# kan-bayashi/espnet

Measured on AMD Instinct MI355X. Metric: frames/sec, 12L Conformer hybrid CTC/attention training step (B=32 T=1000 d=256 per GPU), higher is better.
Workload: dtype f32; 1 GPU; BASELINE configs[1]: 12L Conformer enc d=256 h=4 ff=2048 k=31 macaron+cnn rel_pos, 6L Transformer dec, V=5000, fbank B=32 T=1000 L=100, mtlalpha 0.3, lsm 0.1; global_batch=32, frames=1000, parallelism=dp1, optimizer=adam+noam, clip 5.0, launch=hipGraph, wgrad_side_stream=False, optimizer_steps_done=113

## Files before the change

### espnet_amd/csrc/convmod.hip

```cpp
#include <stdlib.h>
#include "common.h"
#include "../../include/espnet_amd.h"

namespace {

constexpr int KMAX = 32;

__device__ __forceinline__ void chan_merge(float& n, float& mean, float& m2, float nb, float mb, float m2b);

template <int NWV, int MODE>
__global__ __launch_bounds__(NWV * 64) void dwconv_lds_kernel(const float* __restrict__ x, const float* __restrict__ w,
                                                              const float* __restrict__ bias, float* __restrict__ y,
                                                              int B, int T, int C, int K, int pad, int flip,
                                                              const float* __restrict__ aglu, int y_bf16,
                                                              float* __restrict__ bn_part) {
  constexpr int TB = NWV * 8;
  constexpr int NR = (TB + KMAX - 1 + NWV - 1) / NWV;
  constexpr int NWL = (64 * KMAX + NWV * 64 - 1) / (NWV * 64);
  __shared__ float xs[(TB + KMAX - 1) * 64];
  __shared__ float wl[64 * KMAX];
  const int lane = threadIdx.x & 63, wave = threadIdx.x >> 6;
  const int c0 = blockIdx.x * 64;
  const int c = min(c0 + lane, C - 1);
  const int nblk = (T + TB - 1) / TB;
// ... 169 lines not shown
  __syncthreads();
  float* slot = smem + wave * 64 * (KMAX + 1);
#pragma unroll
  for (int k = 0; k < KMAX; ++k)
    if (k < K) slot[lane * (KMAX + 1) + k] = live ? acc[k] : 0.f;
  redb[wave * 64 + lane] = live ? accb : 0.f;
  __syncthreads();
  const int nch = min(64, C - c0);
  for (int i = threadIdx.x; i < nch * K; i += blockDim.x) {
    const int cc = i / K, k = i % K;
    float t = 0.f;
#pragma unroll
    for (int wv = 0; wv < NWV; ++wv) t += smem[wv * 64 * (KMAX + 1) + cc * (KMAX + 1) + k];
    atomicAdd(&dw[(long)c0 * K + i], t);
  }
  if (db && threadIdx.x < nch) {
    float t = 0.f;
#pragma unroll
    for (int wv = 0; wv < NWV; ++wv) t += redb[wv * 64 + threadIdx.x];
    atomicAdd(&db[c0 + threadIdx.x], t);
  }
}

constexpr int BN_R = 4;
struct BnGeom { int cq, rs, slab_rows; };
__host__ __device__ inline BnGeom bn_geom(int C) {
  BnGeom g;
  g.cq = C / 4;
  g.rs = 256 / g.cq;
  g.slab_rows = BN_R * g.rs;
  return g;
}
__device__ __forceinline__ void chan_merge(float& n, float& mean, float& m2, float nb, float mb, float m2b) {
  const float nt = n + nb;
  if (nt > 0.f) {
    const float d = mb - mean;
    const float f = nb / nt;
    mean += d * f;
    m2 += m2b + d * d * n * f;
  }
  n = nt;
}

__global__ __launch_bounds__(256) void bn_partial_kernel(const float* __restrict__ x, float* __restrict__ part,
                                                         long M, int C, int T, const int* __restrict__ bound) {
  __shared__ float4 sh_mean[256], sh_m2[256];
// ... 82 lines not shown
      chan_merge(n, mean, m2, sh[0][o], sh[1][o], sh[2][o]);
    }
    const float var = m2 / n;
    mean_out[c] = mean;
    rstd_out[c] = rsqrtf(var + eps);
    if (running_mean) {
      running_mean[c] = (1.f - momentum) * running_mean[c] + momentum * mean;
      running_var[c] = (1.f - momentum) * running_var[c] + momentum * (n > 1.f ? m2 / (n - 1.f) : var);
    }
  }
}
__global__ void bn_apply_kernel(const float* __restrict__ x, const float* __restrict__ mean,
                                const float* __restrict__ rstd, const float* __restrict__ gamma,
                                const float* __restrict__ beta, float* __restrict__ y, long M, int C, int act,
                                int bf16) {
  const long n = M * C;
  const long stride = (long)gridDim.x * blockDim.x;
  unsigned short* y16 = reinterpret_cast<unsigned short*>(y);
  for (long i = (long)blockIdx.x * blockDim.x + threadIdx.x; i < n; i += stride) {
    int c = i % C;
    float z = (x[i] - mean[c]) * rstd[c] * gamma[c] + beta[c];
    z = eamd_act(z, act);
    if (bf16) y16[i] = eamd_f2bf(z); else y[i] = z;
  }
}
__global__ __launch_bounds__(256) void bn_bwd_partial_kernel(const float* __restrict__ dy, const float* __restrict__ x,
                                                             const float* __restrict__ mean,
                                                             const float* __restrict__ rstd,
                                                             const float* __restrict__ gamma,
                                                             const float* __restrict__ beta, float* __restrict__ part,
                                                             long M, int C, int act, int T,
                                                             const int* __restrict__ bound) {
  __shared__ float4 sh1[256], sh2[256];
  const int tb = bound ? bound[0] : T;
  const BnGeom g = bn_geom(C);
  const int t = threadIdx.x;
  const int q = t % g.cq, sub = t / g.cq;
  const bool live = sub < g.rs;
  const long r0 = (long)blockIdx.x * g.slab_rows + sub;
  float4 mu = make_float4(0.f, 0.f, 0.f, 0.f), rs = mu, gm = mu, be = mu;
  if (live) {
    mu = reinterpret_cast<const float4*>(mean)[q]; rs = reinterpret_cast<const float4*>(rstd)[q];
    gm = reinterpret_cast<const float4*>(gamma)[q]; be = reinterpret_cast<const float4*>(beta)[q];
  }
  float4 xv[BN_R], dv[BN_R];
#pragma unroll
// ... 261 lines not shown
  }
  red[sub][lane] = (s0 + s1) + (s2 + s3);
  __syncthreads();
  if (sub == 0 && col < 10 * C) {
    const float v = (red[0][lane] + red[1][lane]) + (red[2][lane] + red[3][lane]);
    const int k = col / C, c = col % C;
    if (k < 9) atomicAdd(&dw[(long)c * 9 + k], v); else atomicAdd(&db[c], v);
  }
}

inline int grid_for(long n) {
  long b = (n + 255) / 256;
  if (b < 1) b = 1;
  if (b > 4096) b = 4096;
  return (int)b;
}

inline void dwconv_launch(const float* x, const float* w, const float* bias, float* y, int B, int T, int C, int K,
                          int flip, hipStream_t s) {
  hipLaunchKernelGGL((dwconv_lds_kernel<8, 0>), dim3((C + 63) / 64, B * ((T + 63) / 64)), dim3(512), 0, s, x, w, bias, y, B, T, C,
                     K, (K - 1) / 2, flip, (const float*)nullptr, 0, (float*)nullptr);
}

}

extern "C" {

int eamd_dwconv_fwd(const float* x, const float* w, const float* bias, float* y, int B, int T, int C, int K,
                    void* stream) {
  if (!x || !w || !y || B <= 0 || T <= 0 || C <= 0 || K <= 0 || (K & 1) == 0) return EAMD_EINVAL;
  if (K > KMAX) return EAMD_EUNSUPPORTED;
  dwconv_launch(x, w, bias, y, B, T, C, K, 0, (hipStream_t)stream);
  EAMD_LAUNCH_CHECK();
  return EAMD_OK;
}

int eamd_dwconv_bwd_x(const float* dy, const float* w, float* dx, int B, int T, int C, int K, void* stream) {
  if (!dy || !w || !dx || B <= 0 || T <= 0 || C <= 0 || K <= 0 || (K & 1) == 0) return EAMD_EINVAL;
  if (K > KMAX) return EAMD_EUNSUPPORTED;
  dwconv_launch(dy, w, (const float*)nullptr, dx, B, T, C, K, 1, (hipStream_t)stream);
  EAMD_LAUNCH_CHECK();
  return EAMD_OK;
}

int eamd_dwconv_bwd_w(const float* dy, const float* x, float* dw, float* db, int B, int T, int C, int K,
                      void* stream) {
  if (!dy || !x || !dw || B <= 0 || T <= 0 || C <= 0 || K <= 0 || (K & 1) == 0) return EAMD_EINVAL;
  if (K > KMAX) return EAMD_EUNSUPPORTED;
  const long total = (long)B * ((T + WNWV * 8 - 1) / (WNWV * 8));
  const int gx = (C + 63) / 64;
  long gy = (512 + gx - 1) / gx;
  if (gy > total) gy = total;
  if (gy < 1) gy = 1;
  const long tpb = (total + gy - 1) / gy;
  gy = (total + tpb - 1) / tpb;
  hipLaunchKernelGGL(dwconv_bwd_w_kernel, dim3(gx, (unsigned)gy), dim3(WNWV * 64), 0, (hipStream_t)stream, dy, x, dw, db, B,
                     T, C, K, (K - 1) / 2, (int)tpb, 0);
  EAMD_LAUNCH_CHECK();
  return EAMD_OK;
}

int eamd_dwconv_glu_fwd(const float* a, const float* w, const float* bias, float* y, float* bn_part, int B, int T, int C, int K,
                        void* stream) {
  if (!a || !w || !y || B <= 0 || T <= 0 || C <= 0 || K <= 0 || (K & 1) == 0) return EAMD_EINVAL;
  if (K > KMAX) return EAMD_EUNSUPPORTED;
  hipLaunchKernelGGL((dwconv_lds_kernel<8, 1>), dim3((C + 63) / 64, B * ((T + 63) / 64)), dim3(512), 0, (hipStream_t)stream, a, w,
                     bias, y, B, T, C, K, (K - 1) / 2, 0, (const float*)nullptr, 0, bn_part);
  EAMD_LAUNCH_CHECK();
  return EAMD_OK;
}

int eamd_dwconv_glu_bwd_x(const float* dy, const float* w, const float* a, void* da, int da_bf16, int B, int T, int C, int K,
                          void* stream) {
  if (!dy || !w || !a || !da || B <= 0 || T <= 0 || C <= 0 || K <= 0 || (K & 1) == 0) return EAMD_EINVAL;
  if (K > KMAX) return EAMD_EUNSUPPORTED;
  hipLaunchKernelGGL((dwconv_lds_kernel<8, 2>), dim3((C + 63) / 64, B * ((T + 63) / 64)), dim3(512), 0, (hipStream_t)stream, dy, w,
                     (const float*)nullptr, (float*)da, B, T, C, K, (K - 1) / 2, 1, a, da_bf16, (float*)nullptr);
  EAMD_LAUNCH_CHECK();
  return EAMD_OK;
}

int eamd_dwconv_glu_bwd_w(const float* dy, const float* a, float* dw, float* db, int B, int T, int C, int K, void* stream) {
  if (!dy || !a || !dw || B <= 0 || T <= 0 || C <= 0 || K <= 0 || (K & 1) == 0) return EAMD_EINVAL;
  if (K > KMAX) return EAMD_EUNSUPPORTED;
  const long total = (long)B * ((T + WNWV * 8 - 1) / (WNWV * 8));
  const int gx = (C + 63) / 64;
  long gy = (512 + gx - 1) / gx;
  if (gy > total) gy = total;
  if (gy < 1) gy = 1;
  const long tpb = (total + gy - 1) / gy;
  gy = (total + tpb - 1) / tpb;
  hipLaunchKernelGGL(dwconv_bwd_w_kernel, dim3(gx, (unsigned)gy), dim3(WNWV * 64), 0, (hipStream_t)stream, dy, a, dw, db, B,
                     T, C, K, (K - 1) / 2, (int)tpb, 1);
  EAMD_LAUNCH_CHECK();
  return EAMD_OK;
}

static bool bn_shape_ok(int C) { return C >= 4 && C <= 1024 && C % 4 == 0; }
int eamd_bn_nslab(int64_t M, int C) {
  if (!bn_shape_ok(C) || M <= 0) return 0;
  const BnGeom g = bn_geom(C);
  return (int)((M + g.slab_rows - 1) / g.slab_rows);
}

static int bn_stats_impl(const float* x, float* workspace, float* mean, float* rstd, float* running_mean,
                         float* running_var, int64_t* num_batches_tracked, int64_t M, int C, float eps, float momentum, int T,
                         const int32_t* bound, void* stream) {
  if (!x || !workspace || !mean || !rstd || M <= 0 || C <= 0) return EAMD_EINVAL;
  if (bound && (T <= 0 || M % T != 0)) return EAMD_EINVAL;
  if (!bn_shape_ok(C)) return EAMD_EUNSUPPORTED;
  if ((uintptr_t)x & 15) return EAMD_EINVAL;
  hipStream_t s = (hipStream_t)stream;
  const int nslab = eamd_bn_nslab(M, C);
  hipLaunchKernelGGL(bn_partial_kernel, dim3(nslab), dim3(256), 0, s, x, workspace, (long)M, C, T, (const int*)bound);
  EAMD_LAUNCH_CHECK();
  hipLaunchKernelGGL(bn_finalize_kernel, dim3((C + BN_CPB - 1) / BN_CPB), dim3(1024), 0, s, workspace, nslab, C, eps, momentum, mean, rstd,
                     running_mean, running_var, (long long*)num_batches_tracked);
  EAMD_LAUNCH_CHECK();
// ... 2 lines not shown
int eamd_bn_stats(const float* x, float* workspace, float* mean, float* rstd, float* running_mean,
                  float* running_var, int64_t* num_batches_tracked, int64_t M, int C, float eps, float momentum, void* stream) {
  return bn_stats_impl(x, workspace, mean, rstd, running_mean, running_var, num_batches_tracked, M, C, eps, momentum, 1, nullptr, stream);
}
int eamd_bn_stats_bounded(const float* x, float* workspace, float* mean, float* rstd, float* running_mean,
                          float* running_var, int64_t* num_batches_tracked, int64_t M, int C, float eps, float momentum, int T,
                          const int32_t* bound, void* stream) {
  if (!bound) return EAMD_EINVAL;
  return bn_stats_impl(x, workspace, mean, rstd, running_mean, running_var, num_batches_tracked, M, C, eps, momentum, T, bound, stream);
}

int eamd_bn_finalize(const float* part, int nslab, float* mean, float* rstd, float* running_mean, float* running_var,
                     int64_t* num_batches_tracked, int C, float eps, float momentum, void* stream) {
  if (!part || !mean || !rstd || nslab <= 0 || C <= 0) return EAMD_EINVAL;
  hipLaunchKernelGGL(bn_finalize_kernel, dim3((C + BN_CPB - 1) / BN_CPB), dim3(1024), 0, (hipStream_t)stream, part, nslab, C, eps,
                     momentum, mean, rstd, running_mean, running_var, (long long*)num_batches_tracked);
  EAMD_LAUNCH_CHECK();
  return EAMD_OK;
}

int eamd_bn_apply(const float* x, const float* mean, const float* rstd, const float* gamma, const float* beta,
                  void* y, int64_t M, int C, int act, int y_bf16, void* stream) {
  if (!x || !mean || !rstd || !gamma || !beta || !y || M <= 0 || C <= 0) return EAMD_EINVAL;
  hipLaunchKernelGGL(bn_apply_kernel, dim3(grid_for(M * C)), dim3(256), 0, (hipStream_t)stream, x, mean, rstd, gamma,
                     beta, (float*)y, (long)M, C, act, y_bf16);
  EAMD_LAUNCH_CHECK();
  return EAMD_OK;
}

static int bn_bwd_impl(const float* dy, const float* x, const float* mean, const float* rstd, const float* gamma,
                       const float* beta, float* workspace, float* dx, float* dgamma, float* dbeta, int64_t M, int C,
                       int act, int training, int T, const int32_t* bound, void* stream) {
  if (!dy || !x || !mean || !rstd || !gamma || !beta || !workspace || !dx || !dgamma || !dbeta || M <= 0 || C <= 0)
    return EAMD_EINVAL;
  if (bound && (T <= 0 || M % T != 0)) return EAMD_EINVAL;
  if (!bn_shape_ok(C)) return EAMD_EUNSUPPORTED;
  if (((uintptr_t)x | (uintptr_t)dy | (uintptr_t)mean | (uintptr_t)rstd | (uintptr_t)gamma | (uintptr_t)beta) & 15)
    return EAMD_EINVAL;
  hipStream_t s = (hipStream_t)stream;
  const int nslab = eamd_bn_nslab(M, C);
  float* sums = workspace + (long)nslab * 2 * C;
  hipLaunchKernelGGL(bn_bwd_partial_kernel, dim3(nslab), dim3(256), 0, s, dy, x, mean, rstd, gamma, beta,
                     workspace, (long)M, C, act, T, (const int*)bound);
  EAMD_LAUNCH_CHECK();
  hipLaunchKernelGGL(bn_bwd_finalize_kernel, dim3((C + BN_CPB - 1) / BN_CPB), dim3(1024), 0, s, workspace, nslab, C, sums, dgamma, dbeta);
  EAMD_LAUNCH_CHECK();
  hipLaunchKernelGGL(bn_bwd_apply_kernel, dim3(grid_for(M * C)), dim3(256), 0, s, dy, x, mean, rstd, gamma, beta,
                     sums, dx, (long)M, C, act, training, T, (const int*)bound);
  EAMD_LAUNCH_CHECK();
  return EAMD_OK;
}
int eamd_bn_bwd(const float* dy, const float* x, const float* mean, const float* rstd, const float* gamma,
                const float* beta, float* workspace, float* dx, float* dgamma, float* dbeta, int64_t M, int C,
                int act, int training, void* stream) {
  return bn_bwd_impl(dy, x, mean, rstd, gamma, beta, workspace, dx, dgamma, dbeta, M, C, act, training, 1, nullptr, stream);
}
int eamd_bn_bwd_bounded(const float* dy, const float* x, const float* mean, const float* rstd, const float* gamma,
                        const float* beta, float* workspace, float* dx, float* dgamma, float* dbeta, int64_t M, int C,
                        int act, int training, int T, const int32_t* bound, void* stream) {
  if (!bound) return EAMD_EINVAL;
  return bn_bwd_impl(dy, x, mean, rstd, gamma, beta, workspace, dx, dgamma, dbeta, M, C, act, training, T, bound, stream);
}

static int conv_c1_fwd(const float* x, const float* w, const float* bias, void* y, int B, int T, int F, int C,
                       int y_bf16, int st, int pad, void* stream) {
  if (!x || !w || !bias || !y || B <= 0 || T + 2 * pad < 3 || F + 2 * pad < 3 || C <= 0) return EAMD_EINVAL;
  if (F + 2 * pad > C1_MAXF) return EAMD_EUNSUPPORTED;
  int H = (T + 2 * pad - 3) / st + 1, W = (F + 2 * pad - 3) / st + 1;
  hipStream_t s = (hipStream_t)stream;
  const bool pair = y_bf16 && (C % 2 == 0) && (((uintptr_t)y & 3) == 0);
  const int nthr = pair ? ((C / 2 + 63) / 64) * 64 : 256;
#define EAMD_C1F(ST_, NC_) hipLaunchKernelGGL((conv1_fwd_kernel<ST_, NC_>), dim3(B * H), dim3(min(nthr, 256)), 0, s, x, w, \
                                              bias, (float*)y, B, T, F, H, W, C, y_bf16, pad)
  if (st == 2) { if (pair) EAMD_C1F(2, 2); else EAMD_C1F(2, 1); }
  else         { if (pair) EAMD_C1F(1, 2); else EAMD_C1F(1, 1); }
#undef EAMD_C1F
  EAMD_LAUNCH_CHECK();
  return EAMD_OK;
}
int eamd_conv1_fwd(const float* x, const float* w, const float* bias, void* y, int B, int T, int F, int C,
                   int y_bf16, void* stream) {
  return conv_c1_fwd(x, w, bias, y, B, T, F, C, y_bf16, 2, 0, stream);
}
int eamd_conv3x3_c1_fwd(const float* x, const float* w, const float* bias, void* y, int B, int T, int F, int C,
// ... 64 lines not shown
```

### espnet_amd/functional.py

```python
import math

import torch

from . import ops
from .ops import (ACT_NONE, ACT_RELU, ACT_SWISH, EPI_DACT_FACTOR, EPI_MUL_AUX, EPI_MUL_DSWISH, EPI_MUL_RELU_MASK, EPI_NONE,
                  EPI_RELU)


class GradSink:

    on_done = None
    on_use = None

    @staticmethod
    def use(params):
        if GradSink.on_use is not None and torch.is_grad_enabled():
            GradSink.on_use(params)
        return params

    def __init__(self, params):
        self.params = list(params)
        self.ret = [None] * len(self.params)

    def buf(self, i):
# ... 812 lines not shown
        else:
            dq = ops.to_act(dqu)
        kv_in = mem2 if cross else xn
        ops.linear_bwd_w(dq, xn, sink.buf(2), db=sink.buf(3))
        dxn = ops.linear_bwd_x(dq, ops.wshadow(wq))
        dmem = None
        if pre_kv is not None:
            dx = _ln_bwd_out(dxn, x2, ln_w, mean, rstd, do, sink.buf(0), sink.buf(1), ctx.prev, (B, T1, D))
            return (dx, None, None, None, None, None, None, None, None, None) + sink.results()
        ops.linear_bwd_w(dkk, kv_in, sink.buf(4), db=sink.buf(5))
        ops.linear_bwd_w(dv, kv_in, sink.buf(6), db=sink.buf(7))
        if cross:
            dmem = ops.linear_bwd_x(dkk, ops.wshadow(wk))
            ops.linear_bwd_x(dv, ops.wshadow(wv), out=dmem, beta=1.0)
            dmem = dmem.view(B, T2, D)
        else:
            ops.linear_bwd_x(dkk, ops.wshadow(wk), out=dxn, beta=1.0)
            ops.linear_bwd_x(dv, ops.wshadow(wv), out=dxn, beta=1.0)
        dx = _ln_bwd_out(dxn, x2, ln_w, mean, rstd, do, sink.buf(0), sink.buf(1), ctx.prev, (B, T1, D))
        return (dx, dmem, None, None, None, None, None, None, None, None) + sink.results()


FUSE_GLU_DWCONV = True


class ConvModuleBlockFn(torch.autograd.Function):
    @staticmethod
    def forward(ctx, x, running_mean, running_var, training, act, eps, bn_eps, bn_momentum, drop, *params):
        p_out, s_out = drop
        ln_w, ln_b, w1, b1, wd, bd_, g, be, w2, b2 = params
        B, T, D = x.shape
        Cc = w2.shape[0]
        K = wd.shape[-1]
        M = B * T
        adt = ops.act_dtype()
        x2 = x.reshape(M, D).contiguous()
        rp = None
        if eps is not None and D == 256 and Cc == 256 and x2.dtype == torch.float32 and adt == torch.float32 \
                and ops.rowproj_ok(M, D, 2 * Cc) and (p_out <= 0.0 or ops.f32_epilogue_drop()):
            w1v, w2v = w1.detach().view(2 * Cc, D), w2.detach().view(Cc, Cc)
            rp = ops.rowproj_images(w1, [(w1v, False), (w1v, True), (w2v, False), (w2v, True)])
        if rp is not None:
            xn = torch.empty_like(x2)
            mean = torch.empty(M, device=x2.device, dtype=torch.float32)
            rstd = torch.empty_like(mean)
            a = ops.rowproj(xn, rp[0], 2 * Cc, bias=b1, ln=(x2, ln_w, ln_b, eps, mean, rstd))
# ... 36 lines not shown
        ctx.save_for_backward(x2, mean, rstd, xn, a, gl, d, bmean, brstd, e)
        ctx.pr = GradSink.use(params)
        ctx.cfg = (B, T, D, Cc, K, act, training, drop)
        ctx.bound = bound
        ctx.prev = _prev_drop(x)
        return _tag_out(out.view(B, T, D), p_out, s_out)

    @staticmethod
    def backward(ctx, dout):
        x2, mean, rstd, xn, a, gl, d, bmean, brstd, e = ctx.saved_tensors
        ln_w, ln_b, w1, b1, wd, bd_, g, be, w2, b2 = ctx.pr
        B, T, D, Cc, K, act, training, (p_out, s_out) = ctx.cfg
        M = B * T
        adt = ops.act_dtype()
        sink = GradSink(ctx.pr)
        do = dout.reshape(M, D).contiguous()
        dob = _grad_in(dout, do, p_out, s_out)
        rp = ctx.rp
        ops.linear_bwd_w(dob, e, sink.buf(8).view(Cc, Cc), db=sink.buf(9))
        if rp is not None:
            de = ops.rowproj(dob, rp[3], Cc)
        else:
            de = ops.linear_bwd_x(dob, ops.wshadow(w2).view(Cc, Cc))
        dd = ops.bn_bwd(de, d, bmean, brstd, g, be, sink.buf(6), sink.buf(7), M, Cc, act, training, bound=ctx.bound)
        if gl is None:
            da = ops.dwconv_glu_bwd_x(dd, wd.view(Cc, K), a, B, T, Cc, K, adt)
            if ctx.bound is not None:
                ops.mask_time(da, T, ctx.bound[1])
            ops.dwconv_glu_bwd_w(dd, a, sink.buf(4).view(Cc, K), sink.buf(5), B, T, Cc, K)
        else:
            dgl = ops.dwconv_bwd_x(dd, wd.view(Cc, K), B, T, Cc, K)
            ops.dwconv_bwd_w(dd, gl, sink.buf(4).view(Cc, K), sink.buf(5), B, T, Cc, K)
            da = ops.glu_bwd(dgl, a, Cc, adt)
            if ctx.bound is not None:
                ops.mask_time(da, T, ctx.bound[1])
        ops.linear_bwd_w(da, xn, sink.buf(2).view(2 * Cc, D), db=sink.buf(3))
        if rp is not None and da.dtype == torch.float32:
            dx = _rp_ln_bwd(da, rp[1], x2, ln_w, mean, rstd, do, sink.buf(0), sink.buf(1), ctx.prev, (B, T, D))
        else:
            dxn = ops.linear_bwd_x(da, ops.wshadow(w1).view(2 * Cc, D))
            dx = _ln_bwd_out(dxn, x2, ln_w, mean, rstd, do, sink.buf(0), sink.buf(1), ctx.prev, (B, T, D))
        return (dx, None, None, None, None, None, None, None, None) + sink.results()


_TAPS_FWD = [(kh, kw) for kh in range(3) for kw in range(3)]
_CLASSES = [((0, 0), [(0, 0), (0, 2), (2, 0), (2, 2)]), ((0, 1), [(0, 1), (2, 1)]),
            ((1, 0), [(1, 0), (1, 2)]), ((1, 1), [(1, 1)])]


def _conv3s2_fwd(y_in, w, b, B, Hi, Wi, Cc, adt):
    Ho, Wo = (Hi - 3) // 2 + 1, (Wi - 3) // 2 + 1
    wf, wd = ops.conv2_weight_prep(w, adt)
    g = ops.make_gather(Cc, _TAPS_FWD, Ho, Wo, Hi, Wi, 2, 2)
    M = B * Ho * Wo
    y = torch.empty(M, Cc, device=y_in.device, dtype=adt)
    ops.gemm(y_in, wf, y, M, Cc, 9 * Cc, 9 * Cc, Cc, Cc, transB=1, bias=b, epilogue=EPI_RELU, gather=g)
    return y, wd, Ho, Wo

# ... 337 lines not shown
```

### espnet_amd/ops.py

```python
import ctypes as C
import os
import math

import torch

from . import _lib
from ._lib import GatherT, GemmT, RowMapT, check, ptr, stream_ptr

ACT_NONE, ACT_RELU, ACT_SWISH = 0, 1, 2
EPI_NONE, EPI_RELU, EPI_SWISH, EPI_MUL_RELU_MASK, EPI_MUL_DSWISH, EPI_MUL_AUX, EPI_DACT_FACTOR, EPI_ROW_STATS, EPI_ROW_GRAD = 0, 1, 2, 3, 4, 5, 6, 7, 8

_PRECISIONS = {"fp32": 0, "bf16": 1}
_state = {"precision": 0}


def set_precision(name):
    if name not in _PRECISIONS:
        raise ValueError(f"precision must be one of {list(_PRECISIONS)}")
    _state["precision"] = _PRECISIONS[name]


def get_precision():
    return [k for k, v in _PRECISIONS.items() if v == _state["precision"]][0]

# ... 1690 lines not shown
    if bn is None:
        return y
    eps, momentum, running_mean, running_var, nbt = bn
    mean = torch.empty(Cc, device=a.device, dtype=torch.float32)
    rstd = torch.empty(Cc, device=a.device, dtype=torch.float32)
    check(_lib.lib().eamd_bn_finalize(ptr(part), nslab, ptr(mean), ptr(rstd), ptr(running_mean), ptr(running_var), ptr(nbt), Cc,
                                      eps, momentum, stream_ptr()), "eamd_bn_finalize")
    return y, mean, rstd


def dwconv_glu_bwd_x(dy, w, a, B, T, Cc, K, out_dtype=torch.float32):
    da = torch.empty(a.shape, device=a.device, dtype=out_dtype)
    check(_lib.lib().eamd_dwconv_glu_bwd_x(ptr(dy), ptr(w), ptr(a), ptr(da), int(out_dtype == torch.bfloat16), B, T, Cc, K,
                                           stream_ptr()), "eamd_dwconv_glu_bwd_x")
    return da


def dwconv_glu_bwd_w(dy, a, dw, db, B, T, Cc, K):
    assert dw.numel() == Cc * K and (db is None or db.numel() == Cc)
    check(_lib.lib().eamd_dwconv_glu_bwd_w(ptr(dy), ptr(a), ptr(dw), ptr(db), B, T, Cc, K, stream_ptr()),
          "eamd_dwconv_glu_bwd_w")


def bn_stats(x, M, Cc, eps, momentum, running_mean, running_var, num_batches_tracked=None, bound=None):
    nslab = _lib.lib().eamd_bn_nslab(M, Cc)
    ws = torch.empty(3 * Cc * nslab, device=x.device, dtype=torch.float32)
    mean = torch.empty(Cc, device=x.device, dtype=torch.float32)
    rstd = torch.empty(Cc, device=x.device, dtype=torch.float32)
    assert num_batches_tracked is None or (num_batches_tracked.dtype == torch.int64 and num_batches_tracked.is_cuda)
    if bound is not None:
        check(_lib.lib().eamd_bn_stats_bounded(ptr(x), ptr(ws), ptr(mean), ptr(rstd), ptr(running_mean), ptr(running_var),
                                               ptr(num_batches_tracked), M, Cc, eps, momentum,
                                               int(bound[0]), ptr(bound[1]), stream_ptr()), "eamd_bn_stats_bounded")
        return mean, rstd
    check(_lib.lib().eamd_bn_stats(ptr(x), ptr(ws), ptr(mean), ptr(rstd), ptr(running_mean), ptr(running_var),
                                   ptr(num_batches_tracked), M, Cc, eps, momentum, stream_ptr()),
          "eamd_bn_stats")
    return mean, rstd


def bn_apply(x, mean, rstd, gamma, beta, M, Cc, act, out_dtype=torch.float32):
    y = torch.empty(x.shape, device=x.device, dtype=out_dtype)
    check(_lib.lib().eamd_bn_apply(ptr(x), ptr(mean), ptr(rstd), ptr(gamma), ptr(beta), ptr(y), M, Cc,
                                   act, 1 if out_dtype == torch.bfloat16 else 0, stream_ptr()), "eamd_bn_apply")
    return y

# ... 1285 lines not shown
```

### include/espnet_amd.h

```cpp
#ifndef ESPNET_AMD_H_
#define ESPNET_AMD_H_
#include <stdint.h>
#ifdef __cplusplus
extern "C" {
#endif

int eamd_abi_version(void);

typedef struct {
  int32_t enabled;
  int32_t C;
  int32_t ntap;
  int32_t Ho, Wo;
  int32_t Hin, Win;
  int32_t sh, sw;
  int32_t dh[9], dw[9];
} eamd_gather_t;

typedef struct {
  int32_t enabled;
  int32_t Ho, Wo;
  int32_t Hc, Wc;
  int32_t sh, oh, sw, ow;
} eamd_rowmap_t;
// ... 203 lines not shown
                   int64_t pad_idx, void* stream);
int eamd_posenc(const float* x, const float* pe, float* out, int64_t rows, int T, int D, float scale,
                void* stream);
int eamd_posenc_scaled(const float* x, const float* pe, const float* alpha, float* out, int64_t rows, int T, int D,
                       float scale, void* stream);
int eamd_posenc_scaled_bwd(const float* dout, const float* pe, float* dalpha, int64_t rows, int T, int D,
                           void* stream);
int eamd_permute4(const float* src, float* dst, int d0, int d1, int d2, int d3, int64_t s0, int64_t s1,
                  int64_t s2, int64_t s3, int accumulate, void* stream);
int eamd_dropout(const void* x, void* y, int64_t n, float p, const uint64_t* step_dev, uint64_t salt, int act,
                 int in_bf16, int out_bf16, void* stream);
int eamd_rng_advance(uint64_t* step_dev, void* stream);

int eamd_dwconv_fwd(const float* x, const float* w, const float* bias, float* y, int B, int T, int C, int K,
                    void* stream);
int eamd_dwconv_bwd_x(const float* dy, const float* w, float* dx, int B, int T, int C, int K, void* stream);
int eamd_dwconv_bwd_w(const float* dy, const float* x, float* dw, float* db, int B, int T, int C, int K,
                      void* stream);
int eamd_dwconv_glu_fwd(const float* a, const float* w, const float* bias, float* y, float* bn_part, int B, int T, int C, int K,
                        void* stream);
int eamd_dwconv_glu_bwd_x(const float* dy, const float* w, const float* a, void* da, int da_bf16, int B, int T, int C, int K,
                          void* stream);
int eamd_dwconv_glu_bwd_w(const float* dy, const float* a, float* dw, float* db, int B, int T, int C, int K, void* stream);
int eamd_bn_nslab(int64_t M, int C);
int eamd_bn_stats(const float* x, float* workspace, float* mean, float* rstd, float* running_mean,
                  float* running_var, int64_t* num_batches_tracked, int64_t M, int C, float eps, float momentum, void* stream);
int eamd_bn_finalize(const float* part, int nslab, float* mean, float* rstd, float* running_mean, float* running_var,
                     int64_t* num_batches_tracked, int C, float eps, float momentum, void* stream);
int eamd_bn_apply(const float* x, const float* mean, const float* rstd, const float* gamma, const float* beta,
                  void* y, int64_t M, int C, int act, int y_bf16, void* stream);
int eamd_bn_stats_bounded(const float* x, float* workspace, float* mean, float* rstd, float* running_mean,
                          float* running_var, int64_t* num_batches_tracked, int64_t M, int C, float eps, float momentum, int T,
                          const int32_t* bound, void* stream);
int eamd_bn_bwd_bounded(const float* dy, const float* x, const float* mean, const float* rstd, const float* gamma,
                        const float* beta, float* workspace, float* dx, float* dgamma, float* dbeta, int64_t M, int C,
                        int act, int training, int T, const int32_t* bound, void* stream);
int eamd_mask_time(void* x, int64_t rows, int C, int T, const int32_t* bound, int is_bf16, void* stream);
int eamd_bn_bwd(const float* dy, const float* x, const float* mean, const float* rstd, const float* gamma,
                const float* beta, float* workspace, float* dx, float* dgamma, float* dbeta, int64_t M, int C,
                int act, int training, void* stream);
int eamd_conv1_fwd(const float* x, const float* w, const float* bias, void* y, int B, int T, int F, int C,
                   int y_bf16, void* stream);
int64_t eamd_conv1_bwd_w_workspace(int B, int T, int C);
int eamd_conv1_bwd_w(const void* dy, const float* x, float* dw, float* db, float* workspace, int B, int T, int F,
                     int C, int dy_bf16, void* stream);

int64_t eamd_ctc_workspace_bytes(int B, int T, int Lmax);
int eamd_ctc_loss(const float* acts, int64_t stride_t, int64_t stride_b, const int64_t* ys_pad,
                  const int32_t* ilens, float* nll, float* grad, int64_t gstride_t, int64_t gstride_b,
                  void* workspace, int B, int T, int V, int Lmax, int blank, int ignore_id, float grad_scale,
                  void* stream);
int eamd_ctc_grad(const float* acts, int64_t stride_t, int64_t stride_b, const int32_t* ilens, const float* nll, float* grad,
                  int64_t gstride_t, int64_t gstride_b, const void* workspace, int B, int T, int V, int Lmax, int blank,
                  float grad_scale, const float* gscale_dev, void* stream);

int64_t eamd_ctc_pit_workspace_bytes(int S, int B, int T, int Lmax);
int eamd_ctc_pit_loss(const float* acts, const int64_t* ys_pad, const int32_t* ilens, float* nll_pair, int64_t* perm, float* pit,
                      float* grad, void* workspace, int S, int B, int T, int V, int Lmax, int blank, int ignore_id, float grad_scale,
                      void* stream);

// ... 258 lines not shown
```

Measured before the change: 1.143 million frames/s.

## Fuse BN backward apply, depthwise-conv and GLU backward into one conv-module kernel

Adds a templated kernel that applies the batch-norm backward elementwise step on the fly, then computes the depthwise-conv input gradient, the GLU gradient and the weight/bias gradient in one pass. The BN reduction pass still runs separately and now only produces sums. This removes the materialised dd tensor and the separate dwconv bwd_x/bwd_w launches with their re-reads of dy and a. It also adds a float4-vectorised BN apply kernel. The cost is higher register and LDS pressure from the per-K template instantiation, and atomics for dw.

```diff
diff --git a/espnet_amd/csrc/convmod.hip b/espnet_amd/csrc/convmod.hip
--- a/espnet_amd/csrc/convmod.hip
+++ b/espnet_amd/csrc/convmod.hip
@@ -215,6 +215,227 @@
   }
 }
 
+struct BnBwdArgs {
+  const float *x, *mean, *rstd, *gamma, *beta, *sums;
+  const int* bound;
+  long M;
+  int act, training;
+};
+__device__ __forceinline__ float bn_bwd_elem(float x, float dy, float mu, float rs, float g, float be, float s1, float s2,
+                                             float invM, int act, int training) {
+#pragma clang fp contract(off)
+  const float xh = (x - mu) * rs;
+  const float z = __builtin_fmaf(xh, g, be);
+  float d = dy;
+  if (act == EAMD_ACT_SWISH) d *= eamd_dswish(z);
+  else if (act == EAMD_ACT_RELU) d = z > 0.f ? d : 0.f;
+  const float gr = g * rs;
+  if (!training) return gr * d;
+  const float r = __builtin_fmaf(-invM, s1, d);
+  return gr * __builtin_fmaf(-invM, xh * s2, r);
+}
+
+template <int K, int FBN>
+__global__ __launch_bounds__(WNWV * 64, 4) void dwconv_glu_bwd_kernel(const float* __restrict__ dy,
+                                                                   const float* __restrict__ w,
+                                                                   const float* __restrict__ a, float* __restrict__ da,
+                                                                   int da_bf16, float* __restrict__ dw,
+                                                                   float* __restrict__ db, int B, int T, int C,
+                                                                   int pad, int tiles_per_block, BnBwdArgs bn) {
+  constexpr int NWV = WNWV, TB = NWV * 8;
+  constexpr int NR = (TB + K - 1 + NWV - 1) / NWV;
+  constexpr int NJ = 8 + K - 1;
+  __shared__ float smem[NWV * 64 * (KMAX + 1)];
+  static_assert(2 * NR * NWV * 64 <= NWV * 64 * (KMAX + 1), "tiles must fit in the reduction buffer");
+  static_assert(NWV * 8 + K - 1 <= NR * NWV, "a wave's last row must lie inside the tile");
+  float* xs = smem;
+  float* gs = smem + NR * NWV * 64;
+  __shared__ float wl[64 * (KMAX + 1)];
+  __shared__ float redb[NWV * 64];
+  const int lane = threadIdx.x & 63, wave = threadIdx.x >> 6;
+  float* xst = xs + wave * 64 + lane;
+  float* gst = gs + wave * 64 + lane;
+  const float* xrd = xs + wave * 8 * 64 + lane;
+  const float* grd = gs + wave * 8 * 64 + lane;
+  const int c0 = blockIdx.x * 64;
+  const bool live = c0 + lane < C;
+  const int c = live ? c0 + lane : C - 1;
+  const int nblk = (T + TB - 1) / TB;
+  const long total = (long)B * nblk;
+  for (int i = threadIdx.x; i < 64 * (KMAX + 1); i += NWV * 64) {
+    const int cc = i / (KMAX + 1), k = i % (KMAX + 1);
+    wl[i] = (c0 + cc < C && k < K) ? w[(long)(c0 + cc) * K + K - 1 - k] : 0.f;
+  }
+  __shared__ float cst[FBN ? 7 * 64 : 1];
+  int tbn = T;
+  if constexpr (FBN) {
+    tbn = bn.bound ? bn.bound[0] : T;
+    if (wave == 0) {
+      cst[lane] = bn.mean[c]; cst[64 + lane] = bn.rstd[c]; cst[128 + lane] = bn.gamma[c]; cst[192 + lane] = bn.beta[c];
+      cst[256 + lane] = bn.training ? bn.sums[c] : 0.f;
+      cst[320 + lane] = bn.training ? bn.sums[C + c] : 0.f;
+      cst[384 + lane] = bn.bound ? 1.f / ((float)(bn.M / T) * (float)tbn) : 1.f / (float)bn.M;
+    }
+    __syncthreads();
+  }
+  float acc[K];
+#pragma unroll
+  for (int k = 0; k < K; ++k) acc[k] = 0.f;
+  float accb = 0.f;
+  for (int r = 0; r < tiles_per_block; ++r) {
+    const long q = (long)blockIdx.y * tiles_per_block + r;
+    if (q >= total) break;
+    const int b = q / nblk;
+    const int tb0 = (int)(q % nblk) * TB;
+    const float* ab = a + (long)b * T * 2 * C + c;
+    const float* gb = dy + (long)b * T * C + c;
+    float xr[NR], gg[NR], gr[NR];
+    if constexpr (FBN) {
+      const float* xb = bn.x + (long)b * T * C + c;
+      constexpr int NH = (NR + 1) / 2;
+      const float mu = cst[lane], rs = cst[64 + lane], gm = cst[128 + lane], be = cst[192 + lane];
+      const float s1 = cst[256 + lane], s2 = cst[320 + lane], invM = cst[384 + lane];
+#pragma unroll
+      for (int h = 0; h < 2; ++h) {
+        float gq[NH], eq[NH], dq[NH];
+#pragma unroll
+        for (int ii = 0; ii < NH; ++ii) {
+          const int i = h * NH + ii;
+          if (i >= NR) continue;
+          const long ts = min(max(tb0 - pad + wave + i * NWV, 0), T - 1);
+          xr[i] = ab[ts * 2 * C];
+          gq[ii] = ab[ts * 2 * C + C];
+          eq[ii] = gb[ts * C];
+          dq[ii] = xb[ts * C];
+        }
+#pragma unroll
+        for (int ii = 0; ii < NH; ++ii) {
+          const int i = h * NH + ii;
+          if (i >= NR) continue;
+          xr[i] *= eamd_sigmoid(gq[ii]);
+          const float v = bn_bwd_elem(dq[ii], eq[ii], mu, rs, gm, be, s1, s2, invM, bn.act, bn.training);
+          gr[i] = (tb0 - pad + wave + i * NWV < tbn) ? v : 0.f;
+        }
+        __builtin_amdgcn_sched_barrier(0);
+      }
+    } else {
+#pragma unroll
+      for (int i = 0; i < NR; ++i) {
+        const long ts = min(max(tb0 - pad + wave + i * NWV, 0), T - 1);
+        xr[i] = ab[ts * 2 * C];
+        gg[i] = ab[ts * 2 * C + C];
+        gr[i] = gb[ts * C];
+      }
+#pragma unroll
+      for (int i = 0; i < NR; ++i) xr[i] *= eamd_sigmoid(gg[i]);
+    }
+    __syncthreads();
+#pragma unroll
+    for (int i = 0; i < NR; ++i) {
+      const int rr = wave + i * NWV, ts = tb0 - pad + rr;
+      const bool in = ts >= 0 && ts < T;
+      xst[i * NWV * 64] = in ? xr[i] : 0.f;
+      gst[i * NWV * 64] = in ? gr[i] : 0.f;
+    }
+    __syncthreads();
+    const int t0 = tb0 + wave * 8;
+    float dg[8];
+    {
+      float wr[K];
+#pragma unroll
+      for (int k = 0; k < K; ++k) wr[k] = wl[lane * (KMAX + 1) + k];
+#pragma unroll
+      for (int i = 0; i < 8; ++i) dg[i] = 0.f;
+      float vl[NJ];
+#pragma unroll
+      for (int j = 0; j < 8; ++j) vl[j] = grd[j * 64];
+#pragma unroll
+      for (int j0 = 0; j0 < NJ; j0 += 8) {
+#pragma unroll
+        for (int j = j0 + 8; j < j0 + 16; ++j)
+          if (j < NJ) vl[j] = grd[j * 64];
+        __builtin_amdgcn_sched_barrier(0);
+#pragma unroll
+        for (int j = j0; j < j0 + 8; ++j) {
+          if (j >= NJ) continue;
+          const float v = vl[j];
+#pragma unroll
+          for (int i = 0; i < 8; ++i) {
+            const int k = j - i;
+            if (k >= 0 && k < K) dg[i] += wr[k] * v;
+          }
+        }
+#pragma unroll
+        for (int i = 0; i < 8; ++i) asm volatile("" : "+v"(dg[i]));
+        __builtin_amdgcn_sched_barrier(0);
+      }
+    }
+    float av[8], gv[8];
+#pragma unroll
+    for (int i = 0; i < 8; ++i) {
+      const long ro = (long)min(t0 + i, T - 1) * 2 * C;
+      av[i] = ab[ro]; gv[i] = ab[ro + C];
+    }
+    float g[8];
+#pragma unroll
+    for (int i = 0; i < 8; ++i) { g[i] = grd[(pad + i) * 64]; accb += g[i]; }
+    float xl[NJ];
+#pragma unroll
+    for (int j = 0; j < 8; ++j) xl[j] = xrd[j * 64];
+#pragma unroll
+    for (int j0 = 0; j0 < NJ; j0 += 8) {
+#pragma unroll
+      for (int j = j0 + 8; j < j0 + 16; ++j)
+        if (j < NJ) xl[j] = xrd[j * 64];
+      __builtin_amdgcn_sched_barrier(0);
+#pragma unroll
+      for (int j = j0; j < j0 + 8; ++j) {
+        if (j >= NJ) continue;
+        const float xv = xl[j];
+#pragma unroll
+        for (int i = 0; i < 8; ++i) {
+          const int k = j - i;
+          if (k >= 0 && k < K) acc[k] += g[i] * xv;
+        }
+      }
+#pragma unroll
+      for (int k = 0; k < K; ++k) asm volatile("" : "+v"(acc[k]));
+      __builtin_amdgcn_sched_barrier(0);
+    }
+    unsigned short* y16 = reinterpret_cast<unsigned short*>(da) + (long)b * T * 2 * C + c;
+    float* y32 = da + (long)b * T * 2 * C + c;
+#pragma unroll
+    for (int i = 0; i < 8; ++i) {
+      if (!live || t0 + i >= T) continue;
+      const float sg = eamd_sigmoid(gv[i]);
+      const float g1 = dg[i] * sg, g2 = dg[i] * av[i] * sg * (1.f - sg);
+      const long ro = (long)(t0 + i) * 2 * C;
+      if (da_bf16) { y16[ro] = eamd_f2bf(g1); y16[ro + C] = eamd_f2bf(g2); }
+      else { y32[ro] = g1; y32[ro + C] = g2; }
+    }
+  }
+  __syncthreads();
+  float* slot = smem + wave * 64 * (KMAX + 1);
+#pragma unroll
+  for (int k = 0; k < K; ++k) slot[lane * (KMAX + 1) + k] = live ? acc[k] : 0.f;
+  redb[wave * 64 + lane] = live ? accb : 0.f;
+  __syncthreads();
+  const int nch = min(64, C - c0);
+  for (int i = threadIdx.x; i < nch * K; i += blockDim.x) {
+    const int cc = i / K, k = i % K;
+    float t = 0.f;
+#pragma unroll
+    for (int wv = 0; wv < NWV; ++wv) t += smem[wv * 64 * (KMAX + 1) + cc * (KMAX + 1) + k];
+    atomicAdd(&dw[(long)c0 * K + i], t);
+  }
+  if (db && threadIdx.x < nch) {
+    float t = 0.f;
+#pragma unroll
+    for (int wv = 0; wv < NWV; ++wv) t += redb[wv * 64 + threadIdx.x];
+    atomicAdd(&db[c0 + threadIdx.x], t);
+  }
+}
+
 constexpr int BN_R = 4;
 struct BnGeom { int cq, rs, slab_rows; };
 __host__ __device__ inline BnGeom bn_geom(int C) {
@@ -343,6 +564,28 @@
     float z = (x[i] - mean[c]) * rstd[c] * gamma[c] + beta[c];
     z = eamd_act(z, act);
     if (bf16) y16[i] = eamd_f2bf(z); else y[i] = z;
+  }
+}
+__global__ __launch_bounds__(256) void bn_apply_vec_kernel(const float* __restrict__ x, const float* __restrict__ mean,
+                                                           const float* __restrict__ rstd,
+                                                           const float* __restrict__ gamma,
+                                                           const float* __restrict__ beta, float* __restrict__ y, long M,
+                                                           int C, int act, int bf16) {
+  const BnGeom g = bn_geom(C);
+  const int q = threadIdx.x % g.cq, sub = threadIdx.x / g.cq;
+  if (sub >= g.rs) return;
+  const float4 mu = reinterpret_cast<const float4*>(mean)[q], rs = reinterpret_cast<const float4*>(rstd)[q];
+  const float4 gm = reinterpret_cast<const float4*>(gamma)[q], be = reinterpret_cast<const float4*>(beta)[q];
+  unsigned short* y16 = reinterpret_cast<unsigned short*>(y);
+  for (long r = (long)blockIdx.x * g.rs + sub; r < M; r += (long)gridDim.x * g.rs) {
+    const float4 v = reinterpret_cast<const float4*>(x + r * C)[q];
+    float4 z;
+    z.x = eamd_act((v.x - mu.x) * rs.x * gm.x + be.x, act);
+    z.y = eamd_act((v.y - mu.y) * rs.y * gm.y + be.y, act);
+    z.z = eamd_act((v.z - mu.z) * rs.z * gm.z + be.z, act);
+    z.w = eamd_act((v.w - mu.w) * rs.w * gm.w + be.w, act);
+    if (bf16) reinterpret_cast<uint2*>(y16 + r * C)[q] = eamd_pack_bf16x4(z);
+    else reinterpret_cast<float4*>(y + r * C)[q] = z;
   }
 }
 __global__ __launch_bounds__(256) void bn_bwd_partial_kernel(const float* __restrict__ dy, const float* __restrict__ x,
@@ -650,6 +893,38 @@
                      K, (K - 1) / 2, flip, (const float*)nullptr, 0, (float*)nullptr);
 }
 
+dim3 dwconv_bwd_w_grid(int B, int T, int C, int* tpb) {
+  const long total = (long)B * ((T + WNWV * 8 - 1) / (WNWV * 8));
+  const int gx = (C + 63) / 64;
+  long gy = (512 + gx - 1) / gx;
+  if (gy > total) gy = total;
+  if (gy < 1) gy = 1;
+  const long t = (total + gy - 1) / gy;
+  gy = (total + t - 1) / t;
+  *tpb = (int)t;
+  return dim3(gx, (unsigned)gy);
+}
+
+template <int FBN>
+int dwconv_glu_bwd_launch(const float* dy, const float* w, const float* a, void* da, int da_bf16, float* dw, float* db, int B,
+                          int T, int C, int K, const BnBwdArgs& bn, void* stream) {
+  int tpb;
+  const dim3 grid = dwconv_bwd_w_grid(B, T, C, &tpb);
+  switch (K) {
+#define EAMD_DWB(K_)                                                                                                     \
+  case K_:                                                                                                               \
+    hipLaunchKernelGGL((dwconv_glu_bwd_kernel<K_, FBN>), grid, dim3(WNWV * 64), 0, (hipStream_t)stream, dy, w, a,        \
+                       (float*)da, da_bf16, dw, db, B, T, C, (K_ - 1) / 2, tpb, bn);                                     \
+    break;
+    EAMD_DWB(1) EAMD_DWB(3) EAMD_DWB(5) EAMD_DWB(7) EAMD_DWB(9) EAMD_DWB(11) EAMD_DWB(13) EAMD_DWB(15)
+    EAMD_DWB(17) EAMD_DWB(19) EAMD_DWB(21) EAMD_DWB(23) EAMD_DWB(25) EAMD_DWB(27) EAMD_DWB(29) EAMD_DWB(31)
+#undef EAMD_DWB
+  }
+  static_assert(KMAX == 32, "the switch above lists the odd tap counts below KMAX");
+  EAMD_LAUNCH_CHECK();
+  return EAMD_OK;
+}
+
 }
 
 extern "C" {
@@ -675,15 +950,10 @@
                       void* stream) {
   if (!dy || !x || !dw || B <= 0 || T <= 0 || C <= 0 || K <= 0 || (K & 1) == 0) return EAMD_EINVAL;
   if (K > KMAX) return EAMD_EUNSUPPORTED;
-  const long total = (long)B * ((T + WNWV * 8 - 1) / (WNWV * 8));
-  const int gx = (C + 63) / 64;
-  long gy = (512 + gx - 1) / gx;
-  if (gy > total) gy = total;
-  if (gy < 1) gy = 1;
-  const long tpb = (total + gy - 1) / gy;
-  gy = (total + tpb - 1) / tpb;
-  hipLaunchKernelGGL(dwconv_bwd_w_kernel, dim3(gx, (unsigned)gy), dim3(WNWV * 64), 0, (hipStream_t)stream, dy, x, dw, db, B,
-                     T, C, K, (K - 1) / 2, (int)tpb, 0);
+  int tpb;
+  const dim3 grid = dwconv_bwd_w_grid(B, T, C, &tpb);
+  hipLaunchKernelGGL(dwconv_bwd_w_kernel, grid, dim3(WNWV * 64), 0, (hipStream_t)stream, dy, x, dw, db, B,
+                     T, C, K, (K - 1) / 2, tpb, 0);
   EAMD_LAUNCH_CHECK();
   return EAMD_OK;
 }
@@ -711,17 +981,30 @@
 int eamd_dwconv_glu_bwd_w(const float* dy, const float* a, float* dw, float* db, int B, int T, int C, int K, void* stream) {
   if (!dy || !a || !dw || B <= 0 || T <= 0 || C <= 0 || K <= 0 || (K & 1) == 0) return EAMD_EINVAL;
   if (K > KMAX) return EAMD_EUNSUPPORTED;
-  const long total = (long)B * ((T + WNWV * 8 - 1) / (WNWV * 8));
-  const int gx = (C + 63) / 64;
-  long gy = (512 + gx - 1) / gx;
-  if (gy > total) gy = total;
-  if (gy < 1) gy = 1;
-  const long tpb = (total + gy - 1) / gy;
-  gy = (total + tpb - 1) / tpb;
-  hipLaunchKernelGGL(dwconv_bwd_w_kernel, dim3(gx, (unsigned)gy), dim3(WNWV * 64), 0, (hipStream_t)stream, dy, a, dw, db, B,
-                     T, C, K, (K - 1) / 2, (int)tpb, 1);
-  EAMD_LAUNCH_CHECK();
-  return EAMD_OK;
+  int tpb;
+  const dim3 grid = dwconv_bwd_w_grid(B, T, C, &tpb);
+  hipLaunchKernelGGL(dwconv_bwd_w_kernel, grid, dim3(WNWV * 64), 0, (hipStream_t)stream, dy, a, dw, db, B,
+                     T, C, K, (K - 1) / 2, tpb, 1);
+  EAMD_LAUNCH_CHECK();
+  return EAMD_OK;
+}
+
+int eamd_dwconv_glu_bwd(const float* dy, const float* w, const float* a, void* da, int da_bf16, float* dw, float* db, int B,
+                        int T, int C, int K, void* stream) {
+  if (!dy || !w || !a || !da || !dw || B <= 0 || T <= 0 || C <= 0 || K <= 0 || (K & 1) == 0) return EAMD_EINVAL;
+  if (K > KMAX) return EAMD_EUNSUPPORTED;
+  return dwconv_glu_bwd_launch<0>(dy, w, a, da, da_bf16, dw, db, B, T, C, K, BnBwdArgs{}, stream);
+}
+
+int eamd_convmod_bwd(const float* de, const float* d, const float* mean, const float* rstd, const float* gamma,
+                     const float* beta, const float* sums, const float* w, const float* a, void* da, int da_bf16, float* dw,
+                     float* db, int B, int T, int C, int K, int act, int training, const int32_t* bound, void* stream) {
+  if (!de || !d || !mean || !rstd || !gamma || !beta || !sums || !w || !a || !da || !dw || B <= 0 || T <= 0 || C <= 0 ||
+      K <= 0 || (K & 1) == 0)
+    return EAMD_EINVAL;
+  if (K > KMAX || (act != EAMD_ACT_SWISH && act != EAMD_ACT_RELU && act != EAMD_ACT_NONE)) return EAMD_EUNSUPPORTED;
+  const BnBwdArgs bn = {d, mean, rstd, gamma, beta, sums, (const int*)bound, (long)B * T, act, training};
+  return dwconv_glu_bwd_launch<1>(de, w, a, da, da_bf16, dw, db, B, T, C, K, bn, stream);
 }
 
 static bool bn_shape_ok(int C) { return C >= 4 && C <= 1024 && C % 4 == 0; }
@@ -770,6 +1053,14 @@
 int eamd_bn_apply(const float* x, const float* mean, const float* rstd, const float* gamma, const float* beta,
                   void* y, int64_t M, int C, int act, int y_bf16, void* stream) {
   if (!x || !mean || !rstd || !gamma || !beta || !y || M <= 0 || C <= 0) return EAMD_EINVAL;
+  if (bn_shape_ok(C) && !(((uintptr_t)x | (uintptr_t)mean | (uintptr_t)rstd | (uintptr_t)gamma | (uintptr_t)beta |
+                           (uintptr_t)y) & 15)) {
+    const long nb = (M + bn_geom(C).rs - 1) / bn_geom(C).rs;
+    hipLaunchKernelGGL(bn_apply_vec_kernel, dim3((unsigned)(nb < 8192 ? nb : 8192)), dim3(256), 0, (hipStream_t)stream, x,
+                       mean, rstd, gamma, beta, (float*)y, (long)M, C, act, y_bf16);
+    EAMD_LAUNCH_CHECK();
+    return EAMD_OK;
+  }
   hipLaunchKernelGGL(bn_apply_kernel, dim3(grid_for(M * C)), dim3(256), 0, (hipStream_t)stream, x, mean, rstd, gamma,
                      beta, (float*)y, (long)M, C, act, y_bf16);
   EAMD_LAUNCH_CHECK();
@@ -778,8 +1069,8 @@
 
 static int bn_bwd_impl(const float* dy, const float* x, const float* mean, const float* rstd, const float* gamma,
                        const float* beta, float* workspace, float* dx, float* dgamma, float* dbeta, int64_t M, int C,
-                       int act, int training, int T, const int32_t* bound, void* stream) {
-  if (!dy || !x || !mean || !rstd || !gamma || !beta || !workspace || !dx || !dgamma || !dbeta || M <= 0 || C <= 0)
+                       int act, int training, int T, const int32_t* bound, void* stream, bool apply = true) {
+  if (!dy || !x || !mean || !rstd || !gamma || !beta || !workspace || (apply && !dx) || !dgamma || !dbeta || M <= 0 || C <= 0)
     return EAMD_EINVAL;
   if (bound && (T <= 0 || M % T != 0)) return EAMD_EINVAL;
   if (!bn_shape_ok(C)) return EAMD_EUNSUPPORTED;
@@ -793,6 +1084,7 @@
   EAMD_LAUNCH_CHECK();
   hipLaunchKernelGGL(bn_bwd_finalize_kernel, dim3((C + BN_CPB - 1) / BN_CPB), dim3(1024), 0, s, workspace, nslab, C, sums, dgamma, dbeta);
   EAMD_LAUNCH_CHECK();
+  if (!apply) return EAMD_OK;
   hipLaunchKernelGGL(bn_bwd_apply_kernel, dim3(grid_for(M * C)), dim3(256), 0, s, dy, x, mean, rstd, gamma, beta,
                      sums, dx, (long)M, C, act, training, T, (const int*)bound);
   EAMD_LAUNCH_CHECK();
@@ -808,6 +1100,17 @@
                         int act, int training, int T, const int32_t* bound, void* stream) {
   if (!bound) return EAMD_EINVAL;
   return bn_bwd_impl(dy, x, mean, rstd, gamma, beta, workspace, dx, dgamma, dbeta, M, C, act, training, T, bound, stream);
+}
+int eamd_bn_bwd_sums(const float* dy, const float* x, const float* mean, const float* rstd, const float* gamma,
+                     const float* beta, float* workspace, float* dgamma, float* dbeta, int64_t M, int C, int act,
+                     void* stream) {
+  return bn_bwd_impl(dy, x, mean, rstd, gamma, beta, workspace, nullptr, dgamma, dbeta, M, C, act, 1, 1, nullptr, stream, false);
+}
+int eamd_bn_bwd_sums_bounded(const float* dy, const float* x, const float* mean, const float* rstd, const float* gamma,
+                             const float* beta, float* workspace, float* dgamma, float* dbeta, int64_t M, int C, int act,
+                             int T, const int32_t* bound, void* stream) {
+  if (!bound) return EAMD_EINVAL;
+  return bn_bwd_impl(dy, x, mean, rstd, gamma, beta, workspace, nullptr, dgamma, dbeta, M, C, act, 1, T, bound, stream, false);
 }
 
 static int conv_c1_fwd(const float* x, const float* w, const float* bias, void* y, int B, int T, int F, int C,
diff --git a/espnet_amd/functional.py b/espnet_amd/functional.py
--- a/espnet_amd/functional.py
+++ b/espnet_amd/functional.py
@@ -858,6 +858,7 @@
 
 
 FUSE_GLU_DWCONV = True
+FUSE_DWCONV_BWD = 2
 
 
 class ConvModuleBlockFn(torch.autograd.Function):
@@ -940,18 +941,23 @@
             de = ops.rowproj(dob, rp[3], Cc)
         else:
             de = ops.linear_bwd_x(dob, ops.wshadow(w2).view(Cc, Cc))
-        dd = ops.bn_bwd(de, d, bmean, brstd, g, be, sink.buf(6), sink.buf(7), M, Cc, act, training, bound=ctx.bound)
-        if gl is None:
-            da = ops.dwconv_glu_bwd_x(dd, wd.view(Cc, K), a, B, T, Cc, K, adt)
-            if ctx.bound is not None:
-                ops.mask_time(da, T, ctx.bound[1])
-            ops.dwconv_glu_bwd_w(dd, a, sink.buf(4).view(Cc, K), sink.buf(5), B, T, Cc, K)
-        else:
-            dgl = ops.dwconv_bwd_x(dd, wd.view(Cc, K), B, T, Cc, K)
-            ops.dwconv_bwd_w(dd, gl, sink.buf(4).view(Cc, K), sink.buf(5), B, T, Cc, K)
-            da = ops.glu_bwd(dgl, a, Cc, adt)
-            if ctx.bound is not None:
-                ops.mask_time(da, T, ctx.bound[1])
+        da = None
+        if gl is None and FUSE_DWCONV_BWD == 2:
+            da = ops.convmod_bwd(de, d, bmean, brstd, g, be, sink.buf(6), sink.buf(7), wd.view(Cc, K), a, sink.buf(4).view(Cc, K),
+                                 sink.buf(5), B, T, Cc, K, act, training, adt, bound=ctx.bound)
+        if da is None:
+            dd = ops.bn_bwd(de, d, bmean, brstd, g, be, sink.buf(6), sink.buf(7), M, Cc, act, training, bound=ctx.bound)
+            if gl is not None:
+                dgl = ops.dwconv_bwd_x(dd, wd.view(Cc, K), B, T, Cc, K)
+                ops.dwconv_bwd_w(dd, gl, sink.buf(4).view(Cc, K), sink.buf(5), B, T, Cc, K)
+                da = ops.glu_bwd(dgl, a, Cc, adt)
+            elif FUSE_DWCONV_BWD:
+                da = ops.dwconv_glu_bwd(dd, wd.view(Cc, K), a, sink.buf(4).view(Cc, K), sink.buf(5), B, T, Cc, K, adt)
+            else:
+                da = ops.dwconv_glu_bwd_x(dd, wd.view(Cc, K), a, B, T, Cc, K, adt)
+                ops.dwconv_glu_bwd_w(dd, a, sink.buf(4).view(Cc, K), sink.buf(5), B, T, Cc, K)
+        if ctx.bound is not None:
+            ops.mask_time(da, T, ctx.bound[1])
         ops.linear_bwd_w(da, xn, sink.buf(2).view(2 * Cc, D), db=sink.buf(3))
         if rp is not None and da.dtype == torch.float32:
             dx = _rp_ln_bwd(da, rp[1], x2, ln_w, mean, rstd, do, sink.buf(0), sink.buf(1), ctx.prev, (B, T, D))
diff --git a/espnet_amd/ops.py b/espnet_amd/ops.py
--- a/espnet_amd/ops.py
+++ b/espnet_amd/ops.py
@@ -1736,6 +1736,37 @@
           "eamd_dwconv_glu_bwd_w")
 
 
+def dwconv_glu_bwd(dd, w, a, dw, db, B, T, Cc, K, out_dtype=torch.float32):
+    assert dw.numel() == Cc * K and (db is None or db.numel() == Cc)
+    da = torch.empty(a.shape, device=a.device, dtype=out_dtype)
+    check(_lib.lib().eamd_dwconv_glu_bwd(ptr(dd), ptr(w), ptr(a), ptr(da), int(out_dtype == torch.bfloat16), ptr(dw), ptr(db),
+                                         B, T, Cc, K, stream_ptr()), "eamd_dwconv_glu_bwd")
+    return da
+
+
+def convmod_bwd(de, d, mean, rstd, gamma, beta, dgamma, dbeta, w, a, dw, db, B, T, Cc, K, act, training,
+                out_dtype=torch.float32, bound=None):
+    if act not in (0, 1, 2):
+        return None
+    M = B * T
+    L = _lib.lib()
+    nslab = L.eamd_bn_nslab(M, Cc)
+    ws = torch.empty((2 * nslab + 2) * Cc, device=d.device, dtype=torch.float32)
+    sums = ws[2 * nslab * Cc:]
+    da = torch.empty(a.shape, device=a.device, dtype=out_dtype)
+    if bound is not None:
+        check(L.eamd_bn_bwd_sums_bounded(ptr(de), ptr(d), ptr(mean), ptr(rstd), ptr(gamma), ptr(beta), ptr(ws), ptr(dgamma),
+                                         ptr(dbeta), M, Cc, act, int(bound[0]), ptr(bound[1]), stream_ptr()),
+              "eamd_bn_bwd_sums_bounded")
+    else:
+        check(L.eamd_bn_bwd_sums(ptr(de), ptr(d), ptr(mean), ptr(rstd), ptr(gamma), ptr(beta), ptr(ws), ptr(dgamma), ptr(dbeta),
+                                 M, Cc, act, stream_ptr()), "eamd_bn_bwd_sums")
+    check(L.eamd_convmod_bwd(ptr(de), ptr(d), ptr(mean), ptr(rstd), ptr(gamma), ptr(beta), ptr(sums), ptr(w), ptr(a), ptr(da),
+                             int(out_dtype == torch.bfloat16), ptr(dw), ptr(db), B, T, Cc, K, act, int(training),
+                             ptr(bound[1]) if bound is not None else None, stream_ptr()), "eamd_convmod_bwd")
+    return da
+
+
 def bn_stats(x, M, Cc, eps, momentum, running_mean, running_var, num_batches_tracked=None, bound=None):
     nslab = _lib.lib().eamd_bn_nslab(M, Cc)
     ws = torch.empty(3 * Cc * nslab, device=x.device, dtype=torch.float32)
diff --git a/include/espnet_amd.h b/include/espnet_amd.h
--- a/include/espnet_amd.h
+++ b/include/espnet_amd.h
@@ -249,6 +249,11 @@
 int eamd_dwconv_glu_bwd_x(const float* dy, const float* w, const float* a, void* da, int da_bf16, int B, int T, int C, int K,
                           void* stream);
 int eamd_dwconv_glu_bwd_w(const float* dy, const float* a, float* dw, float* db, int B, int T, int C, int K, void* stream);
+int eamd_dwconv_glu_bwd(const float* dy, const float* w, const float* a, void* da, int da_bf16, float* dw, float* db, int B,
+                        int T, int C, int K, void* stream);
+int eamd_convmod_bwd(const float* de, const float* d, const float* mean, const float* rstd, const float* gamma,
+                     const float* beta, const float* sums, const float* w, const float* a, void* da, int da_bf16, float* dw,
+                     float* db, int B, int T, int C, int K, int act, int training, const int32_t* bound, void* stream);
 int eamd_bn_nslab(int64_t M, int C);
 int eamd_bn_stats(const float* x, float* workspace, float* mean, float* rstd, float* running_mean,
                   float* running_var, int64_t* num_batches_tracked, int64_t M, int C, float eps, float momentum, void* stream);
@@ -263,6 +268,12 @@
                         const float* beta, float* workspace, float* dx, float* dgamma, float* dbeta, int64_t M, int C,
                         int act, int training, int T, const int32_t* bound, void* stream);
 int eamd_mask_time(void* x, int64_t rows, int C, int T, const int32_t* bound, int is_bf16, void* stream);
+int eamd_bn_bwd_sums(const float* dy, const float* x, const float* mean, const float* rstd, const float* gamma,
+                     const float* beta, float* workspace, float* dgamma, float* dbeta, int64_t M, int C, int act,
+                     void* stream);
+int eamd_bn_bwd_sums_bounded(const float* dy, const float* x, const float* mean, const float* rstd, const float* gamma,
+                             const float* beta, float* workspace, float* dgamma, float* dbeta, int64_t M, int C, int act,
+                             int T, const int32_t* bound, void* stream);
 int eamd_bn_bwd(const float* dy, const float* x, const float* mean, const float* rstd, const float* gamma,
                 const float* beta, float* workspace, float* dx, float* dgamma, float* dbeta, int64_t M, int C,
                 int act, int training, void* stream);
```

Measured after the change: 1.151 million frames/s (median of 6 runs). Within noise of the previous version (+0.7%).
